# tky823/ssspy

Hardware: AMD Instinct MI355X
Metric: GaussILRMA-IP1 update_once mixture-iterations/sec (F=1025,T=512,N=4,K=16) (higher is better)
Workload: dtype f64; 1 GPU; BASELINE configs[1] GaussILRMA-IP1/MM (N=M=4, F=1025, T=512, n_basis=16) x 128 independent mixtures per GPU (configs[4] shard), record_loss=False, update_once() = one fused C-ABI call; batch_per_gpu=128, global_batch=128, n_bins=1025, n_frames=512, n_basis=16, parallelism=mixtures sharded, no collective, input=nmf_mixture(seed=1000+b) per mixture b (SURVEY 8d)

## Files before the change

### include/ssspy_amd.h

```cpp
#ifndef SSSPY_AMD_H
#define SSSPY_AMD_H

#include <stddef.h>

#ifdef __cplusplus
extern "C" {
#endif

enum {
  SSSPY_OK = 0,
  SSSPY_ERR_BADARG = 1,
  SSSPY_ERR_HIP = 2,
  SSSPY_ERR_UNSUPPORTED = 3,
  SSSPY_ERR_INTERNAL = 4,
};

enum { SSSPY_FLOOR_NONE = 0, SSSPY_FLOOR_MAX = 1, SSSPY_FLOOR_ADD = 2 };

enum {
  SSSPY_WEIGHT_UNIT = 0,
  SSSPY_WEIGHT_FRAME = 1,
  SSSPY_WEIGHT_BIN_FRAME = 2,
};

// ... 185 lines not shown
int ssspy_ilrma_deferred_logdet_slots(int B, int N, int F, int T, int K, double domain,
                                      int source_model);
int ssspy_ilrma_ip1_update_loss_slots(const void *X, const void *C, void *W, double *basis,
                                      double *activation, void *U, int B, int N, int F, int T,
                                      int K, double domain, int source_model, double model_param,
                                      int normalize, int floor_kind, double floor_eps,
                                      void *workspace, size_t workspace_bytes, int *info,
                                      double *slots, long long slot_stride, double *logdet,
                                      void *stream);
size_t ssspy_fold_scalar_slots_workspace_bytes(long long total, int nslots);
int ssspy_fold_scalar_slots(const double *slots, long long total, int nslots, double *out,
                            void *workspace, size_t workspace_bytes, void *stream);

enum {
  SSSPY_ROUTE_LATENCY = 0,
  SSSPY_ROUTE_THROUGHPUT = 1,
  SSSPY_ROUTE_GROUPED = 2,
  SSSPY_ROUTE_GENERIC = 3,
  SSSPY_ROUTE_WIDE_BASIS = 4,
  SSSPY_ROUTE_RUNTIME_N = 5,
};
int ssspy_ilrma_route(int B, int N, int F, int T, int K, double domain, int source_model,
                      int *act_chunks, int *basis_plan);

int ssspy_ipa_sweep(void *Vc, void *G, int B, int F, int N, int normalization, int max_iter,
                    int floor_kind, double floor_eps, int *info, void *newton_ws,
                    int *not_converged, void *stream);
size_t ssspy_ipa_sweep_newton_words(int B, int N);
int ssspy_debug_barrier_timeouts(void);

int ssspy_ilrma_partition_expand(const double *basis, const double *activation,
                                 const double *latent, double *Teff, double *Vrep, int B, int N,
                                 int F, int T, int K, void *stream);

enum { SSSPY_PARTITION_LATENT = 1, SSSPY_PARTITION_BASIS = 2, SSSPY_PARTITION_ACTIVATION = 4 };

int ssspy_ilrma_partition_update(const void *X, const void *W, double *basis, double *activation,
                                 double *latent, double *Teff, double *Vrep, int B, int N, int F,
                                 int T, int K, double domain, int source_model, double model_param,
                                 int steps, int floor_kind, double floor_eps, void *workspace,
                                 size_t workspace_bytes, void *stream);

int ssspy_ilrma_partition_normalize(void *W, const void *C, void *Y, double *basis, double *latent,
                                    int B, int N, int F, int T, int K, double domain,
                                    int floor_kind, double floor_eps, void *workspace,
                                    size_t workspace_bytes, void *stream);
// ... 585 lines not shown
```

### ssspy_amd/_lib.py

```python

import ctypes
import os

import numpy as np

_PKG = os.path.dirname(os.path.abspath(__file__))
LIB_PATH = os.environ.get("SSSPY_AMD_LIB") or os.path.join(_PKG, "lib", "libssspy_amd.so")

OK, ERR_BADARG, ERR_HIP, ERR_UNSUPPORTED, ERR_INTERNAL = 0, 1, 2, 3, 4
FLOOR_NONE, FLOOR_MAX, FLOOR_ADD = 0, 1, 2
WEIGHT_UNIT, WEIGHT_FRAME, WEIGHT_BIN_FRAME = 0, 1, 2
SOURCE_GAUSS, SOURCE_T, SOURCE_GGD = 0, 1, 2
PARTITION_LATENT, PARTITION_BASIS, PARTITION_ACTIVATION = 1, 2, 4
SOURCE_ME = 0x100
CONTRAST_LAPLACE, CONTRAST_GAUSS, CONTRAST_GAUSS_FIXED = 0, 1, 2
WHITEN, PCA_FIRST_COMPONENT_LAST, PCA_FIRST_COMPONENT_FIRST = 0, 1, 2
IPSDTA_QUAD, IPSDTA_BASIS, IPSDTA_ACT, IPSDTA_COV = range(4)
IPSDTA_MAX_SOURCES, IPSDTA_MAX_BLOCK, IPSDTA_MAX_BASIS = 8, 8, 32
(ROUTE_LATENCY, ROUTE_THROUGHPUT, ROUTE_GROUPED, ROUTE_GENERIC, ROUTE_WIDE_BASIS,
 ROUTE_RUNTIME_N) = range(6)
MNMF_ROUTE_TILED, MNMF_ROUTE_GENERIC, MNMF_ROUTE_RUNTIME = range(3)
MNMF_PLAN_FIELDS = ("fast", "ksmall", "basis_copy", "glds_cov", "glds_spatial", "kq", "handover",
                    "tail_full", "tail_tail", "tail_split", "tail_groups", "htail_full", "htail_tail",
                    "htail_split", "htail_groups", "act_chunks", "ip1_records", "spatial_fold_in_norm",
# ... 81 lines not shown
    "ssspy_ilrma_weighted_covariance": (_i, [_p, _p, _p, _p, _p, _i, _i, _i, _i, _i, _d, _i, _d, _i,
                                             _d, _p, _z, _p]),
    "ssspy_ilrma_normalize_filter": (_i, [_p, _p, _p, _i, _i, _i, _i, _d, _i, _d, _p, _z, _p]),
    "ssspy_ilrma_normalize_output": (_i, [_p, _p, _p, _i, _i, _i, _i, _i, _d, _i, _d, _p, _z, _p]),
    "ssspy_ilrma_normalize_output_tracked": (_i, [_p, _p, _p, _i, _i, _i, _i, _i, _d, _i, _d, _p, _z,
                                                  _p, _p]),
    "ssspy_ilrma_iss_weight": (_i, [_p, _p, _p, _p, _i, _i, _i, _i, _i, _d, _i, _d, _i, _d, _p]),
    "ssspy_ilrma_iss_weight_power": (_i, [_p, _p, _p, _p, _i, _i, _i, _i, _i, _d, _i, _d, _i, _d, _p]),
    "ssspy_ilrma_loss_workspace_bytes": (_z, [_i, _i, _i, _i, _i, _i]),
    "ssspy_ilrma_loss_data": (_i, [_p, _p, _p, _p, _p, _i, _i, _i, _i, _i, _d, _i, _d, _p, _z, _p]),
    "ssspy_ilrma_ip1_update": (_i, [_p, _p, _p, _p, _p, _p, _i, _i, _i, _i, _i, _d, _i, _d, _i, _i, _d,
                                    _p, _z, _p, _p]),
    "ssspy_ilrma_deferred_loss_supported": (_i, [_i, _i, _i, _i, _d, _i]),
    "ssspy_ilrma_ip1_update_deferred_loss": (_i, [_p, _p, _p, _p, _p, _p, _i, _i, _i, _i, _i, _d, _i,
                                                  _d, _i, _i, _d, _p, _z, _p, _p, _p, _p]),
    "ssspy_ilrma_deferred_loss_slots": (_i, [_i, _i, _i, _i, _i, _d, _i]),
    "ssspy_ilrma_deferred_logdet_slots": (_i, [_i, _i, _i, _i, _i, _d, _i]),
    "ssspy_ilrma_ip1_update_loss_slots": (_i, [_p, _p, _p, _p, _p, _p, _i, _i, _i, _i, _i, _d, _i,
                                               _d, _i, _i, _d, _p, _z, _p, _p, _q, _p, _p]),
    "ssspy_fold_scalar_slots_workspace_bytes": (_z, [_q, _i]),
    "ssspy_fold_scalar_slots": (_i, [_p, _q, _i, _p, _p, _z, _p]),
    "ssspy_ilrma_route": (_i, [_i, _i, _i, _i, _i, _d, _i, ctypes.POINTER(ctypes.c_int),
                                ctypes.POINTER(ctypes.c_int)]),
    "ssspy_ilrma_partition_expand": (_i, [_p, _p, _p, _p, _p, _i, _i, _i, _i, _i, _p]),
    "ssspy_ilrma_partition_update": (_i, [_p, _p, _p, _p, _p, _p, _p, _i, _i, _i, _i, _i, _d, _i, _d,
                                          _i, _i, _d, _p, _z, _p]),
    "ssspy_ilrma_partition_normalize": (_i, [_p, _p, _p, _p, _p, _i, _i, _i, _i, _i, _d, _i, _d, _p,
                                             _z, _p]),
    "ssspy_iva_frame_power_workspace_bytes": (_z, [_i, _i, _i, _i]),
    "ssspy_iva_frame_power": (_i, [_p, _p, _p, _i, _i, _i, _i, _p, _z, _p]),
    "ssspy_separate_frame_power": (_i, [_p, _p, _p, _p, _i, _i, _i, _i, _p, _z, _p]),
    "ssspy_iva_weight": (_i, [_p, _p, _p, _i, _i, _i, _i, _i, _i, _d, _p]),
    "ssspy_iva_loss_data": (_i, [_p, _p, _p, _i, _i, _i, _i, _i, _p]),
    "ssspy_overiva_frame_power_workspace_bytes": (_z, [_i, _i, _i, _i]),
    "ssspy_overiva_frame_power": (_i, [_p, _p, _q, _p, _p, _i, _i, _i, _i, _i, _p, _z, _p]),
    "ssspy_overiva_step_workspace_bytes": (_z, [_i, _i]),
    "ssspy_overiva_step": (_i, [_p, _p, _p, _i, _i, _i, _i, _i, _d, _p, _p, _p, _p, _z, _p]),
    "ssspy_iva_score_weight": (_i, [_p, _p, _p, _i, _i, _i, _i, _i, _i, _d, _p]),
    "ssspy_iva_grad_step_logdet_slots": (_i, [_i, _i, _i]),
    "ssspy_iva_grad_step": (_i, [_p, _p, _i, _i, _i, _i, _i, _i, _d, _p, _p, _q, _p]),
    "ssspy_fdica_weight": (_i, [_p, _p, _i, _i, _i, _i, _i, _i, _d, _p, _q, _p]),
    "ssspy_fdica_route": (_i, [_i, _i, _i, _i, _i]),
    "ssspy_fdica_steps": (_i, [_p, _p, _i, _i, _i, _i, _i, _i, _d, _i, _d, _i, _p, _p, _q, _p, _p]),
    "ssspy_wpe_route": (_i, [_i, _i, _i, _i, _i, ctypes.POINTER(ctypes.c_int)]),
    "ssspy_wpe_steps": (_i, [_p, _p, _p, _i, _i, _i, _i, _i, _i, _i, _d, _i, _p, _q, _p, _i, _p]),
    "ssspy_wpe_step": (_i, [_p, _p, _p, _i, _i, _i, _i, _i, _i, _i, _d, _p, _p, _p, _p, _p, _i, _p]),
# ... 182 lines not shown
```

### ssspy_amd/_ops.py

```python

from . import _device as dv
from . import _lib, _routes
from ._device import ptr


def _L():
    return _lib.load()


import os as _os

_CANARY_DOUBLES = 4096 if _os.environ.get("SSSPY_AMD_WS_CANARY") else 0
_CANARY_VALUE = -7.25e300
_canaries = []


def _workspace(nbytes, dev):
    n = (int(nbytes) + 7) // 8
    buf = dv.empty((n + _CANARY_DOUBLES,), dv.f64, dev)
    if not _CANARY_DOUBLES:
        return buf, int(nbytes)
    import weakref

    buf[n:].fill_(_CANARY_VALUE)
# ... 499 lines not shown
        ptr(X), ptr(C), ptr(W), ptr(basis), ptr(activation), ptr(U), B, N, F, T, K, domain, model[0],
        model[1], int(bool(normalize)), flooring[0], flooring[1], ptr(ws), ws_bytes, ptr(info),
        ptr(slots), int(slot_stride), ptr(logdet), _st()), "ilrma_ip1_update_loss_slots")


def fold_scalar_slots(slots, total, nslots, out):
    ws, ws_bytes = _scratch(_L().ssspy_fold_scalar_slots_workspace_bytes(int(total), int(nslots)),
                            slots.device)
    _lib.check(_L().ssspy_fold_scalar_slots(ptr(slots), int(total), int(nslots), ptr(out), ptr(ws),
                                            ws_bytes, _st()), "fold_scalar_slots")
    return out


def ilrma_route(B, N, F, T, K, domain, model=GAUSS):
    import ctypes

    chunks = ctypes.c_int(0)
    plan = (ctypes.c_int * 3)()
    route = int(_L().ssspy_ilrma_route(B, N, F, T, K, float(domain), model[0], ctypes.byref(chunks),
                                       plan))
    if route < 0:
        raise ValueError("ilrma_route: bad shape")
    return route, int(chunks.value), tuple(plan)


def ilrma_partition_expand(basis, activation, latent, Teff, Vrep):
    B, N, F, K = Teff.shape
    T = Vrep.shape[-1]
    _lib.check(
        _L().ssspy_ilrma_partition_expand(ptr(basis), ptr(activation), ptr(latent), ptr(Teff),
                                          ptr(Vrep), B, N, F, T, K, _st()),
        "ilrma_partition_expand",
    )


def ilrma_partition_update(X, W, basis, activation, latent, Teff, Vrep, domain, steps, flooring, ws,
                           ws_bytes, model=GAUSS):
    B, N, F, T = X.shape
    K = basis.shape[-1]
    _lib.check(
        _L().ssspy_ilrma_partition_update(ptr(X), ptr(W), ptr(basis), ptr(activation), ptr(latent),
                                          ptr(Teff), ptr(Vrep), B, N, F, T, K, domain, model[0],
                                          model[1], steps, flooring[0], flooring[1], ptr(ws),
                                          ws_bytes, _st()),
        "ilrma_partition_update",
    )
# ... 1328 lines not shown
```

### ssspy_amd/csrc/ilrma_api.hip

```cpp
#include "ilrma_plan.hpp"

namespace ssspy {

static inline int check_model(int source_model, double param, double domain = 2.0) {
  const int model = source_model & 0xff;
  const bool me = (source_model & SSSPY_SOURCE_ME) != 0;
  if ((source_model & ~(0xff | SSSPY_SOURCE_ME)) != 0)
    return fail(SSSPY_ERR_BADARG, "bad source model flags");
  if (me && (domain != 2.0 || model == SSSPY_SOURCE_GGD))
    return fail(SSSPY_ERR_BADARG, "ME source updates need domain == 2 and a Gauss or t model");
  if (model == SSSPY_SOURCE_GAUSS) return SSSPY_OK;
  if (model == SSSPY_SOURCE_T && param > 0.0) return SSSPY_OK;
  if (model == SSSPY_SOURCE_GGD && param > 0.0 && param < 2.0) return SSSPY_OK;
  return fail(SSSPY_ERR_BADARG, "bad source model / model_param (t: dof > 0, GGD: 0 < beta < 2)");
}

int ip1_with_power(void *W, const void *U, const void *C, double *qbuf, int B, int F, int N,
                   int floor_kind, double floor_eps, int *info, hipStream_t st);
int separate_power(const void *X, const void *W, double *P, int B, int N, int F, int T,
                   hipStream_t st);
int row_power(const void *W, const void *C, double *qbuf, int B, int F, int N, hipStream_t st);
int wb_update_basis(const double *a, const double *b, double *basis, const double *activation,
                    double *nd, int BN, int F, int T, int K, const IlrmaDims &d, hipStream_t st);
int wb_update_activation(const double *a, const double *b, const double *basis, double *activation,
// ... 772 lines not shown
    int split = 0, rbins = 0;
    auto cov = [&]() -> int {
      ILRMA_FAST_DISPATCH(N, ilrma_fast_wcov, X, W, basis, activation, U, B, F, T, K, ws + w.upart,
                          p.fm_id, p.fm_param, floor_kind, floor_eps, st, &split, &rbins);
    };
    rc = cov();
    if (rc) return rc;
    auto ip1 = [&]() -> int {
      if (loss_data && loss_stride > 0) {
        ILRMA_FAST_DISPATCH(N, ilrma_small_ip1_logdet,
                            split ? (const void *)(ws + w.upart) : (const void *)U, split, rbins, 0ll,
                            normalize ? C : nullptr, W, B, F, floor_kind, floor_eps, qbuf, info,
                            logdet, loss_stride, st);
      }
      ILRMA_FAST_DISPATCH(N, ilrma_small_ip1, split ? (const void *)(ws + w.upart) : (const void *)U,
                          split, rbins, 0ll, normalize ? C : nullptr, W, B, F, floor_kind, floor_eps,
                          qbuf, info, st);
    };
    rc = ip1();
    if (rc || !normalize) return rc;
    ILRMA_FAST_DISPATCH(N, ilrma_small_norm, W, basis, qbuf, B, F, K, domain, floor_kind, floor_eps,
                        st);
  }
  rc = wcov_into(p, w, d, X, W, basis, activation, U, ws, p.power_once ? Xs : nullptr, p.power_once,
                 st);
  if (rc) return rc;
  rc = ip1_with_power(W, U, normalize ? C : nullptr, normalize ? qbuf : nullptr, B, F, N,
                      floor_kind, floor_eps, info, st);
  if (rc || !normalize) return rc;
  return launch_norm_scale(W, basis, qbuf, B, N, F, K, domain, floor_kind, floor_eps, st);
}

int ssspy_ilrma_ip1_update(const void *X, const void *C, void *W, double *basis, double *activation,
                           void *U, int B, int N, int F, int T, int K, double domain,
                           int source_model, double model_param, int normalize, int floor_kind,
                           double floor_eps, void *workspace, size_t workspace_bytes, int *info,
                           void *stream) {
  return ip1_update_impl(X, C, W, basis, activation, U, B, N, F, T, K, domain, source_model,
                         model_param, normalize, floor_kind, floor_eps, workspace, workspace_bytes,
                         info, nullptr, nullptr, stream);
}

int ssspy_ilrma_deferred_loss_supported(int N, int F, int T, int K, double domain,
                                        int source_model) {
  return make_ilrma_plan(1, N, F, T, K, domain, source_model).loss_byproduct;
}
// ... 27 lines not shown
                                      void *workspace, size_t workspace_bytes, int *info,
                                      double *slots, long long slot_stride, double *logdet,
                                      void *stream) {
  SSSPY_REQUIRE(slots && logdet && slot_stride >= B && slot_stride < (1ll << 31),
                "ilrma_ip1_update_loss_slots: bad argument");
  return ip1_update_impl(X, C, W, basis, activation, U, B, N, F, T, K, domain, source_model,
                         model_param, normalize, floor_kind, floor_eps, workspace, workspace_bytes,
                         info, slots, logdet, stream, slot_stride);
}

int ssspy_ilrma_route(int B, int N, int F, int T, int K, double domain, int source_model,
                      int *chunks_out, int *basis_plan) {
  if (B <= 0 || N < 2 || N > SSSPY_RT_MAX_SOURCES || F <= 0 || T <= 0 || K < 1 ||
      K > SSSPY_MAX_BASIS || !(domain > 0.0 && domain <= 2.0))
    return -1;
  const IlrmaPlan p = make_ilrma_plan(B, N, F, T, K, domain, source_model);
  if (chunks_out) *chunks_out = p.act_chunks;
  if (basis_plan) {
    basis_plan[0] = p.basis_tail.full;
    basis_plan[1] = p.basis_tail.tail;
    basis_plan[2] = p.basis_tail.split;
  }
  return p.summary;
}

size_t ssspy_fold_scalar_slots_workspace_bytes(long long total, int nslots) {
  if (total <= 0 || nslots <= 0) return 0;
  return align256(fold_scratch_bytes(total, nslots)) + 256;
}

int ssspy_fold_scalar_slots(const double *slots, long long total, int nslots, double *out,
                            void *workspace, size_t workspace_bytes, void *stream) {
  SSSPY_REQUIRE(slots && out && total > 0 && nslots > 0, "fold_scalar_slots: bad argument");
  SSSPY_REQUIRE(workspace && workspace_bytes >= ssspy_fold_scalar_slots_workspace_bytes(total, nslots),
                "fold_scalar_slots: workspace too small");
  return launch_fold_slabs(slots, workspace, out, total, nslots, as_stream(stream), 0);
}

int ssspy_ilrma_partition_expand(const double *basis, const double *activation,
                                 const double *latent, double *Teff, double *Vrep, int B, int N,
                                 int F, int T, int K, void *stream) {
  SSSPY_REQUIRE(basis && activation && latent && Teff && Vrep && B > 0 && N >= 1 && F > 0 &&
                    T > 0 && K >= 1,
                "partition_expand: bad argument");
  const long long per = (long long)K * (F > T ? F : T);
  hipLaunchKernelGGL(k_partition_expand, dim3((unsigned)((per + 255) / 256), N, B), dim3(256), 0,
// ... 106 lines not shown
```

### ssspy_amd/csrc/ilrma_fast.hip

```cpp
#include <cstdlib>

#include "common.hpp"
#include "cov_core.hpp"
#include "fast_model.hpp"
#include "fast_tiles.hpp"
#include "tail_plan.hpp"

#ifndef SSSPY_N
#error "compile with -DSSSPY_N=<n_sources>"
#endif
#if SSSPY_N > 4
#error "fast path is built for n_sources <= 4"
#endif

#define SSSPY_CAT_(a, b) a##b
#define SSSPY_CAT(a, b) SSSPY_CAT_(a, b)
#define LAUNCHER(name) SSSPY_CAT(SSSPY_CAT(name, _n), SSSPY_N)

namespace ssspy {
namespace SSSPY_CAT(ilrma_fast_n, SSSPY_N) {

constexpr int N = SSSPY_N;
using fast::rcp_nr;
using fast::FastModel;
using fast::FM_GAUSS;
using fast::FM_GAUSS1;
using fast::FM_GAUSSP;
using fast::FM_GGD;
// ... 431 lines not shown
}

template <int G>
__device__ __forceinline__ void wc_half_tile(double (&acc)[4][WC_HALF], const c128 *patch,
                                             const double *shared, int lane, int c, int q) {
#pragma unroll
  for (int r = 0; r < 4; ++r) {
    c128 x[4];
#pragma unroll
    for (int m = 0; m < 4; ++m) x[m] = patch[(m * 16 + c) * 17 + q + 4 * r];
    double phi[4];
#pragma unroll
    for (int n = 0; n < 4; ++n)
      phi[n] = shared[(n * 4 + r) * 64 + lane];
    double v[WC_HALF];
    wc_half_terms<G>(x, v);
#pragma unroll
    for (int n = 0; n < 4; ++n)
#pragma unroll
      for (int e = 0; e < WC_HALF; ++e) acc[n][e] = fma(phi[n], v[e], acc[n][e]);
  }
}

template <int G>
__device__ __forceinline__ void wc_half_store(const double (&acc)[4][WC_HALF], c128 *dst,
                                              double scale) {
  constexpr int PA[2][4][2] = {{{0, 1}, {2, 3}, {0, 0}, {0, 0}}, {{0, 2}, {0, 3}, {1, 2}, {1, 3}}};
  constexpr int NPAIR = G == 0 ? 2 : 4, P0 = G == 0 ? 4 : 0;
#pragma unroll
  for (int n = 0; n < 4; ++n) {
    c128 *d = dst + n * 16;
    if constexpr (G == 0) {
#pragma unroll
      for (int a = 0; a < 4; ++a) d[a * 4 + a] = cmake(acc[n][a] * scale, 0.0);
    }
#pragma unroll
    for (int p = 0; p < NPAIR; ++p) {
      const int a = PA[G][p][0], bb = PA[G][p][1];
      const double zx = acc[n][P0 + 2 * p], zy = acc[n][P0 + 2 * p + 1];
      d[a * 4 + bb] = cmake(zx * scale, zy * scale);
      d[bb * 4 + a] = cmake(zx * scale, -zy * scale);
    }
  }
}

template <int MODEL, int KS, bool FULL = false>
__global__ __launch_bounds__(256, KS >= 16 ? 1 : 2) void k_wcov_fast(const c128 *__restrict__ X,
                                                      const c128 *__restrict__ W,
                                                      const double *__restrict__ basis,
                                                      const double *__restrict__ act,
                                                      c128 *__restrict__ U, int F, int T, int K,
                                                      TailPlan plan, c128 *__restrict__ upart,
                                                      FastModel fm) {
  constexpr int SG = WC_SG;
  constexpr int WSTRIDE = N * N + 1;
  __shared__ __attribute__((aligned(16))) c128 xpatch[4][XPATCH];
  constexpr bool NEEDS_Y = MODEL == FM_T || MODEL == FM_GGD;
  __shared__ __attribute__((aligned(16))) c128 wlc[NEEDS_Y ? 4 * 16 * WSTRIDE : 1];
  constexpr bool SPLIT = WC_SHARE && !NEEDS_Y && MODEL != FM_GAUSSP && KS == 4;
  __shared__ __attribute__((aligned(16))) double phis[SPLIT ? WC_WB * N * 4 * 64 : 1];
  const int lane = threadIdx.x & 63, wave = threadIdx.x >> 6;
  const int c = lane & 15, q = lane >> 4;
  const BlockWork work = block_work(plan);
  const int b = work.b, nchunks = work.nchunks;
  const int g = wave % WC_NG, wb = wave / WC_NG;
  const int s0 = g * SG;
  const int i0 = (work.group * WC_WB + wb) * 16;
  const int bin = min(i0 + c, F - 1);
  const fast::XSrc<N> xsrc = fast::make_xsrc<N>(X + (long long)b * N * F * T, F, T);
  c128 *xshare = &xpatch[0][0] + wb * (N * 16 * 17);
  const double *act_b = act + (long long)b * N * K * T;
  const int ntiles = (T + 15) >> 4;
  const int tpc = (ntiles + nchunks - 1) / nchunks;
  const int jt_begin = work.chunk * tpc, jt_end = min(ntiles, jt_begin + tpc);
  if (wave_idle(i0, F)) {
    if (NEEDS_Y) __syncthreads();
    if constexpr (WC_SHARE) {
      for (int jt = jt_begin; jt < jt_end; ++jt) {
        __syncthreads();
        __syncthreads();
      }
    }
    return;
  }
  double tb[SG][KS];
#pragma unroll
  for (int s = 0; s < SG; ++s)
#pragma unroll
    for (int ks = 0; ks < KS; ++ks) {
      const int kk = 4 * ks + q, n = min(s0 + s, N - 1);
      tb[s][ks] = (FULL || kk < K) ? basis[(((long long)b * N + n) * F + bin) * K + kk] : 0.0;
    }
  c128 *wmine = wlc + (NEEDS_Y ? (wave * 16 + c) * WSTRIDE : 0);
  if (NEEDS_Y) {
    for (int e = lane; e < 16 * N * N; e += 64) {
      const int bl = e / (N * N), rem = e % (N * N);
      wlc[(wave * 16 + bl) * WSTRIDE + rem] = W[((long long)b * F + min(i0 + bl, F - 1)) * (N * N) + rem];
    }
  }
  CovAcc<N, SPLIT ? 1 : SG> acc;
  double hacc[SPLIT ? 4 : 1][WC_HALF];
  if constexpr (SPLIT) {
#pragma unroll
    for (int n = 0; n < 4; ++n)
#pragma unroll
// ... 92 lines not shown
    }
  }
  const double scale = 1.0 / (double)T;
  const int ob = i0 + c;
  auto out_bin = [&]() -> c128 * {
    return nchunks == 1 ? U + ((long long)b * F + ob) * (long long)(N * N * N)
                        : upart + (((long long)work.tail_idx * nchunks + work.chunk) * WC_BINS +
                                   (ob - work.group * WC_BINS)) * (long long)(N * N * N);
  };
  if constexpr (SPLIT) {
#pragma unroll
    for (int n = 0; n < 4; ++n)
#pragma unroll
      for (int e = 0; e < WC_HALF; ++e) {
        double v = hacc[n][e];
        v += __shfl_xor(v, 16, 64);
        v += __shfl_xor(v, 32, 64);
        hacc[n][e] = v;
      }
    if (ob < F && q == 0) {
      c128 *dst = out_bin();
      if (gu == 0) wc_half_store<0>(hacc, dst, scale);
      else wc_half_store<1>(hacc, dst, scale);
    }
    return;
  }
  acc.fold_q();
  if (ob < F) {
    c128 *dst = out_bin();
#pragma unroll
    for (int s = 0; s < SG; ++s) {
      const int n = s0 + s;
      if (n < N) {
        int e = 0;
#pragma unroll
        for (int a = 0; a < N; ++a) {
          const bool mine = (a & 3) == q;
          if (mine) dst[(n * N + a) * N + a] = cmake(acc.diag[s][a] * scale, 0.0);
#pragma unroll
          for (int bb = a + 1; bb < N; ++bb) {
            const c128 z = acc.off[s][e];
            if (mine) {
              dst[(n * N + a) * N + bb] = cmake(z.x * scale, z.y * scale);
              dst[(n * N + bb) * N + a] = cmake(z.x * scale, -z.y * scale);
            }
            ++e;
// ... 62 lines not shown
  if (ob < F) {
    c128 *dst = U + ((long long)b * F + ob) * (long long)(N * N * N);
#pragma unroll
    for (int s = 0; s < SG; ++s) {
      const int n = s0 + s;
      if (n < N) {
        int e = 0;
#pragma unroll
        for (int a = 0; a < N; ++a) {
          const bool mine = (a & 3) == q;
          if (mine) dst[(n * N + a) * N + a] = cmake(acc.diag[s][a] * scale, 0.0);
#pragma unroll
          for (int bb = a + 1; bb < N; ++bb) {
            const c128 z = acc.off[s][e];
            if (mine) {
              dst[(n * N + a) * N + bb] = cmake(z.x * scale, z.y * scale);
              dst[(n * N + bb) * N + a] = cmake(z.x * scale, -z.y * scale);
            }
            ++e;
          }
        }
      }
    }
  }
}

__global__ __launch_bounds__(256) void k_wcov_fold(c128 *__restrict__ U,
                                                   const c128 *__restrict__ upart, int F,
                                                   TailPlan plan) {
  constexpr int PER = WC_BINS * N * N * N;
  const int tail_idx = blockIdx.y;
  const int item = plan.full + tail_idx;
  const int b = item / plan.groups, group = item - b * plan.groups;
  const int e = blockIdx.x * blockDim.x + threadIdx.x;
  const int lb = e / (N * N * N);
  if (e >= PER || group * WC_BINS + lb >= F) return;
  const c128 s2 = ordered_sum(upart + (long long)tail_idx * plan.split * PER + e, (long long)PER,
                              plan.split);
  U[((long long)b * F + group * WC_BINS) * (long long)(N * N * N) + e] = s2;
}

template <int KS>
struct TStage {
  double t[(N * 16 * 4 * KS + 255) / 256];
  c128 w;
};
// ... 393 lines not shown
  const int nslots = plan.groups * (plan.split > 1 ? plan.split : 1) * 4;
  int rc = scalar_slots_begin(loss_ws, B, nslots, st);
  if (rc) return rc;
  double *slots = (double *)loss_ws;
  SSSPY_FAST_LAUNCH2(k_loss_fast, W != nullptr, (const c128 *)X, (const c128 *)W,
                     basis, act, slots, F, T, K, plan, fm, B);
  rc = check_launch("k_loss_fast");
  return rc ? rc : scalar_slots_fold(loss_ws, B, nslots, out, 0, st);
}

int LAUNCHER(ilrma_fast_wcov)(const void *X, const void *W, const double *basis, const double *act,
                              void *U, int B, int F, int T, int K, void *upart, int fmodel,
                              double mparam, int floor_kind, double floor_eps, hipStream_t st,
                              int *split_out = nullptr, int *rbins_out = nullptr) {
  if (split_out) *split_out = 0;
  if (rbins_out) *rbins_out = WC_BINS;
  const TailPlan plan =
      make_tail_plan(B, (F + WC_BINS - 1) / WC_BINS, (T + 15) / 16, K > 32 ? 256 : SLOTS,
                     K > 32 ? 256 : 1024);
  const FastModel fm = make_fast_model(fmodel, mparam, 0, floor_kind, floor_eps);
  dim3 grid(plan.full + plan.tail * plan.split), block(256);
#define SSSPY_WCOV_LAUNCH_F(M, KS_, FULL_)                                                        \
  hipLaunchKernelGGL((k_wcov_fast<M, KS_, FULL_>), grid, block, 0, st, (const c128 *)X,            \
                     (const c128 *)W, basis, act, (c128 *)U, F, T, K, plan, (c128 *)upart, fm)
#define SSSPY_WCOV_LAUNCH(M, KS_) SSSPY_WCOV_LAUNCH_F(M, KS_, false)
#define SSSPY_WCOV_LAUNCH_M(KS_)                       \
  switch (fmodel) {                                    \
    case FM_T: SSSPY_WCOV_LAUNCH(FM_T, KS_); break;    \
    case FM_GGD: SSSPY_WCOV_LAUNCH(FM_GGD, KS_); break; \
    case FM_GAUSS1: SSSPY_WCOV_LAUNCH(FM_GAUSS1, KS_); break; \
    case FM_GAUSSP: SSSPY_WCOV_LAUNCH(FM_GAUSSP, KS_); break; \
    default: SSSPY_WCOV_LAUNCH(FM_GAUSS, KS_); break;  \
  }
  if (K > 32) {
    SSSPY_WCOV_LAUNCH_M(16)
  } else if (K > 16) {
    SSSPY_WCOV_LAUNCH_M(8)
  } else if (full_tiles(K, T) && fmodel == FM_GAUSS) {
    SSSPY_WCOV_LAUNCH_F(FM_GAUSS, 4, true);
  } else {
    SSSPY_WCOV_LAUNCH_M(4)
  }
#undef SSSPY_WCOV_LAUNCH_M
#undef SSSPY_WCOV_LAUNCH
#undef SSSPY_WCOV_LAUNCH_F
  int rc = check_launch("k_wcov_fast");
  if (rc || plan.tail == 0) return rc;
  if (split_out && plan.full == 0) {
    *split_out = plan.split;
    return rc;
  }
  hipLaunchKernelGGL(k_wcov_fold, dim3((WC_BINS * N * N * N + 255) / 256, plan.tail), block, 0, st,
                     (c128 *)U, (const c128 *)upart, F, plan);
  return check_launch("k_wcov_fold");
}

int LAUNCHER(ilrma_fast_wcov_frame)(const void *X, const double *weight, void *U, int B, int F,
                                    int T, hipStream_t st) {
  static const bool disabled = std::getenv("SSSPY_AMD_NO_FAST") != nullptr;
  const int groups = (F + WC_BINS - 1) / WC_BINS;
  const long long items = (long long)B * groups;
  if (disabled || items < SLOTS || (long long)F * T * 16 >= (1ll << 32)) return -1;
  hipLaunchKernelGGL(k_wcov_frame_fast, dim3((unsigned)items), dim3(256), 0, st, (const c128 *)X,
                     weight, (c128 *)U, F, T, groups);
  return check_launch("k_wcov_frame_fast");
}

#endif

#undef SSSPY_FAST_LAUNCH2
#undef SSSPY_FAST_LAUNCH_M

}
```

### ssspy_amd/csrc/ilrma_plan.hpp

```cpp
#pragma once

#include <cstdlib>

#include "common.hpp"
#include "ilrma_params.hpp"
#include "tail_plan.hpp"
#include "wide_n.hpp"

namespace ssspy {

#define DECL_N(n)                                                                               \
  int ilrma_basis_n##n(const void *, const void *, const double *, double *, const double *,   \
                       IlrmaDims, hipStream_t);                                                \
  int ilrma_activation_n##n(const void *, const void *, const double *, const double *, double *, \
                            int, IlrmaDims, hipStream_t);                                      \
  int ilrma_wcov_n##n(const void *, const void *, const double *, const double *, void *,       \
                      IlrmaDims, hipStream_t);                                                 \
  size_t ilrma_loss_ws_bytes_n##n(int, int);                                                   \
  int ilrma_loss_n##n(const void *, const void *, const double *, const double *, double *,     \
                      void *, IlrmaDims, hipStream_t);
DECL_N(2) DECL_N(3) DECL_N(4) DECL_N(5) DECL_N(6) DECL_N(7) DECL_N(8)
#undef DECL_N

#define DECL_FAST(n)                                                                           \
  int ilrma_fast_basis_n##n(const void *, const void *, const double *, double *, const double *, \
                            int, int, int, int, int, double, double *, int, double, int,        \
                            double *, void *, int, hipStream_t, long long);                     \
  int ilrma_fast_basis_loss_slots_n##n(int, int, int);                                          \
  size_t ilrma_fast_loss_ws_bytes_n##n(int, int);                                               \
  int ilrma_fast_activation_n##n(const void *, const void *, const double *, double *,         \
                                 double *, int, int, int, int, int, int, double, int,           \
                                 hipStream_t, int *, int, int, double);                         \
  int ilrma_fast_wcov_n##n(const void *, const void *, const double *, const double *, void *, \
                           int, int, int, int, void *, int, double, int, double, hipStream_t,  \
                           int *, int *);                                                      \
  int ilrma_fast_loss_n##n(const void *, const void *, const double *, const double *, double *, \
                           void *, int, int, int, int, int, double, hipStream_t);
DECL_FAST(2) DECL_FAST(3) DECL_FAST(4)
#undef DECL_FAST

#define DECL_SMALL(n)                                                                           \
  size_t ilrma_small_scratch_n##n(int, int, int, int);                                            \
  int ilrma_small_activation_n##n(const void *, const void *, const double *, double *, int, int, \
                                  int, int, int, double, double *, int, double, int,              \
                                  hipStream_t);                                                   \
  int ilrma_small_ip1_n##n(const void *, int, int, long long, const void *, void *, int, int, int, \
                           double, double *, int *, hipStream_t);                                 \
  int ilrma_small_ip1_logdet_n##n(const void *, int, int, long long, const void *, void *, int,   \
                                  int, int, double, double *, int *, double *, long long,         \
                                  hipStream_t);                                                   \
  int ilrma_small_norm_n##n(void *, double *, const double *, int, int, int, double, int, double, \
                            hipStream_t);
DECL_SMALL(2) DECL_SMALL(3) DECL_SMALL(4)
#undef DECL_SMALL

bool wide_weighted_cov_ok(int N, int S, int F, int T, int kind);
int wide_weighted_cov(const void *A, const double *weight, int kind, void *U, int B, int N, int S,
                      int F, int T, hipStream_t st);
size_t wb_loss_ws_bytes(int B, int N, int F, int T);

#define ILRMA_FAST_DISPATCH(N_, fn, ...)             \
  switch (N_) {                                      \
    case 2: return fn##_n2(__VA_ARGS__);             \
    case 3: return fn##_n3(__VA_ARGS__);             \
    default: return fn##_n4(__VA_ARGS__);            \
  }
#define ILRMA_DISPATCH_OR(N_, otherwise, fn, ...)                                    \
  switch (N_) {                                                                      \
    case 2: return fn##_n2(__VA_ARGS__);                                             \
    case 3: return fn##_n3(__VA_ARGS__);                                             \
    case 4: return fn##_n4(__VA_ARGS__);                                             \
    case 5: return fn##_n5(__VA_ARGS__);                                             \
    case 6: return fn##_n6(__VA_ARGS__);                                             \
    case 7: return fn##_n7(__VA_ARGS__);                                             \
    case 8: return fn##_n8(__VA_ARGS__);                                             \
    default: return otherwise;                                                       \
  }
#define ILRMA_DISPATCH(N_, fn, ...)                                                               \
  ILRMA_DISPATCH_OR(N_, fail(SSSPY_ERR_UNSUPPORTED, "ILRMA: n_sources must be in [2, 8]"), fn, \
                    __VA_ARGS__)

static inline bool tuned_sources(int N) { return N >= 2 && N <= 4; }
// ... 92 lines not shown
enum class CovRoute { RuntimeN, WideBasis, MatrixCore, Tuned, Generic };

struct IlrmaPlan {
  int N, K;
  int fm_id, me;
  double fm_param;
  bool gauss;
  NmfRoute nmf;
  SourceRun runs[3];
  int nruns;
  int act_chunks;
  bool act_latency;
  bool act_in_place;
  bool basis_out_of_place;
  TailPlan basis_tail;
  LossRoute loss;
  bool loss_byproduct;
  int loss_slots, logdet_slots;
  bool runtime_n;
  bool cov_matrix_core;
  bool cov_tuned;
  bool power_once;
  bool ip1_latency;
  bool weights_buf;
  bool dense_buf;
  int summary;
};

static inline IlrmaPlan make_ilrma_plan(int B, int N, int F, int T, int K, double domain,
                                        int source_model, double model_param = 0.0) {
  IlrmaPlan p;
  p.N = N;
  p.K = K;
  p.fm_id = fast_model_id(domain, source_model);
  p.fm_param = p.fm_id == 4 ? domain : model_param;
  p.me = (source_model & SSSPY_SOURCE_ME) ? 1 : 0;
  p.gauss = (source_model & 0xff) == SSSPY_SOURCE_GAUSS;
  const bool fast = fast_path(N, F, T, K, domain, source_model);
  const bool small = small_path(B, N, F, T, K, domain, source_model);
  const bool wide = wide_basis_shape(N, K);
  p.nruns = source_runs(B, N, F, T, K, domain, source_model, p.runs);
  p.nmf = p.nruns               ? NmfRoute::Grouped
          : (fast && K <= 32)   ? NmfRoute::Tuned
          : wide                ? NmfRoute::WideBasis
                                : NmfRoute::Generic;
  const bool tuned = p.nmf == NmfRoute::Tuned;
  p.act_chunks = act_chunks(B, N, F, T, K);
  p.act_latency = small;
#ifdef SSSPY_NO_ACT_INPLACE
  p.act_in_place = false;
#else
  p.act_in_place = tuned && p.act_chunks == 1 && K <= 16;
#endif
  p.basis_out_of_place = K > 16;
  p.basis_tail = tuned ? ilrma_basis_plan(B, F, T, K) : TailPlan{0, 0, 1, 0};
  p.runtime_n = rt_sources_ok(N);
  p.loss = (fast && K <= 16)           ? LossRoute::Tuned
           : (K > 16 || p.runtime_n)   ? LossRoute::WideBasis
                                       : LossRoute::Generic;
  p.loss_byproduct = p.loss == LossRoute::Tuned && p.fm_id != 1;
  p.loss_slots = p.loss_byproduct ? tuned_basis_loss_slots(B, N, F, T) : 0;
  p.logdet_slots = p.loss_byproduct ? (small ? (F + 15) / 16 : 1) : 0;
  p.cov_matrix_core = N > 4 && wide_weighted_cov_ok(N, N, F, T, SSSPY_WEIGHT_BIN_FRAME);
  p.cov_tuned = fast;
  p.power_once = p.nmf == NmfRoute::Grouped || p.nmf == NmfRoute::WideBasis;
  p.ip1_latency = small;
  p.weights_buf = N > 4 || wide;
  p.dense_buf = wide;
  p.summary = p.runtime_n                      ? SSSPY_ROUTE_RUNTIME_N
              : p.nmf == NmfRoute::Grouped     ? SSSPY_ROUTE_GROUPED
              : small                          ? SSSPY_ROUTE_LATENCY
              : p.nmf == NmfRoute::WideBasis   ? SSSPY_ROUTE_WIDE_BASIS
              : tuned                          ? SSSPY_ROUTE_THROUGHPUT
                                               : SSSPY_ROUTE_GENERIC;
  return p;
}

static inline CovRoute cov_route(const IlrmaPlan &p, bool ysep, bool filter) {
  const bool weights_ok = p.gauss || ysep || !filter;
  if (p.runtime_n) return CovRoute::RuntimeN;
  if (p.K > 32 && weights_ok) return CovRoute::WideBasis;
  if (p.cov_matrix_core && weights_ok) return CovRoute::MatrixCore;
  if (p.cov_tuned && (p.gauss || filter)) return CovRoute::Tuned;
  return CovRoute::Generic;
}

static inline IlrmaPlan shape_plan(int B, int N, int F, int T, int K) {
  return make_ilrma_plan(B, N, F, T, K, 2.0, SSSPY_SOURCE_GAUSS);
}
// ... 56 lines not shown
```

Measured before the change: 42390 iterations/s.

## Fuse the IP1 demixing update into the weighted covariance kernel epilogue

For the tuned Gauss N=4 route, the weighted covariance kernel now stages each bin's U matrices in shared memory and runs the IP1 row solve in place, writing W and the normalisation powers directly. Bins handled by split tail tiles are finished by a separate small kernel after the fold. This removes the round trip of U through global memory and the separate IP1 launch. In exchange it adds extra barriers and shared-memory reuse inside the covariance kernel, plus a new per-row pivoting solver built from lane shuffles.

```diff
diff --git a/include/ssspy_amd.h b/include/ssspy_amd.h
--- a/include/ssspy_amd.h
+++ b/include/ssspy_amd.h
@@ -231,6 +231,8 @@
 };
 int ssspy_ilrma_route(int B, int N, int F, int T, int K, double domain, int source_model,
                       int *act_chunks, int *basis_plan);
+int ssspy_ilrma_ip1_route(int B, int N, int F, int T, int K, double domain, int source_model,
+                          int *cov_plan);
 
 int ssspy_ipa_sweep(void *Vc, void *G, int B, int F, int N, int normalization, int max_iter,
                     int floor_kind, double floor_eps, int *info, void *newton_ws,
diff --git a/ssspy_amd/_lib.py b/ssspy_amd/_lib.py
--- a/ssspy_amd/_lib.py
+++ b/ssspy_amd/_lib.py
@@ -127,6 +127,7 @@
     "ssspy_fold_scalar_slots": (_i, [_p, _q, _i, _p, _p, _z, _p]),
     "ssspy_ilrma_route": (_i, [_i, _i, _i, _i, _i, _d, _i, ctypes.POINTER(ctypes.c_int),
                                 ctypes.POINTER(ctypes.c_int)]),
+    "ssspy_ilrma_ip1_route": (_i, [_i, _i, _i, _i, _i, _d, _i, ctypes.POINTER(ctypes.c_int)]),
     "ssspy_ilrma_partition_expand": (_i, [_p, _p, _p, _p, _p, _i, _i, _i, _i, _i, _p]),
     "ssspy_ilrma_partition_update": (_i, [_p, _p, _p, _p, _p, _p, _p, _i, _i, _i, _i, _i, _d, _i, _d,
                                           _i, _i, _d, _p, _z, _p]),
diff --git a/ssspy_amd/_ops.py b/ssspy_amd/_ops.py
--- a/ssspy_amd/_ops.py
+++ b/ssspy_amd/_ops.py
@@ -545,6 +545,16 @@
     if route < 0:
         raise ValueError("ilrma_route: bad shape")
     return route, int(chunks.value), tuple(plan)
+
+
+def ilrma_ip1_route(B, N, F, T, K, domain, model=GAUSS):
+    import ctypes
+
+    plan = (ctypes.c_int * 3)()
+    epi = int(_L().ssspy_ilrma_ip1_route(B, N, F, T, K, float(domain), model[0], plan))
+    if epi < 0:
+        raise ValueError("ilrma_ip1_route: bad shape")
+    return bool(epi), tuple(plan)
 
 
 def ilrma_partition_expand(basis, activation, latent, Teff, Vrep):
diff --git a/ssspy_amd/csrc/ilrma_api.hip b/ssspy_amd/csrc/ilrma_api.hip
--- a/ssspy_amd/csrc/ilrma_api.hip
+++ b/ssspy_amd/csrc/ilrma_api.hip
@@ -818,6 +818,12 @@
     ILRMA_FAST_DISPATCH(N, ilrma_small_norm, W, basis, qbuf, B, F, K, domain, floor_kind, floor_eps,
                         st);
   }
+  if (p.cov_ip1_epilogue) {
+    rc = ilrma_fast_wcov_ip1_n4(X, W, normalize ? C : nullptr, basis, activation, U, B, F, T, K,
+                                ws + w.upart, p.fm_id, floor_kind, floor_eps, qbuf, info, st);
+    if (rc || !normalize) return rc;
+    return launch_norm_scale(W, basis, qbuf, B, N, F, K, domain, floor_kind, floor_eps, st);
+  }
   rc = wcov_into(p, w, d, X, W, basis, activation, U, ws, p.power_once ? Xs : nullptr, p.power_once,
                  st);
   if (rc) return rc;
@@ -891,6 +897,18 @@
     basis_plan[2] = p.basis_tail.split;
   }
   return p.summary;
+}
+
+int ssspy_ilrma_ip1_route(int B, int N, int F, int T, int K, double domain, int source_model,
+                          int *cov_plan) {
+  if (ssspy_ilrma_route(B, N, F, T, K, domain, source_model, nullptr, nullptr) < 0) return -1;
+  const IlrmaPlan p = make_ilrma_plan(B, N, F, T, K, domain, source_model);
+  if (cov_plan) {
+    cov_plan[0] = p.cov_tail.full;
+    cov_plan[1] = p.cov_tail.tail;
+    cov_plan[2] = p.cov_tail.split;
+  }
+  return p.cov_ip1_epilogue ? 1 : 0;
 }
 
 size_t ssspy_fold_scalar_slots_workspace_bytes(long long total, int nslots) {
diff --git a/ssspy_amd/csrc/ilrma_fast.hip b/ssspy_amd/csrc/ilrma_fast.hip
--- a/ssspy_amd/csrc/ilrma_fast.hip
+++ b/ssspy_amd/csrc/ilrma_fast.hip
@@ -4,6 +4,7 @@
 #include "cov_core.hpp"
 #include "fast_model.hpp"
 #include "fast_tiles.hpp"
+#include "ip1_rows_exact.hpp"
 #include "tail_plan.hpp"
 
 #ifndef SSSPY_N
@@ -481,14 +482,14 @@
   }
 }
 
-template <int G>
+template <int G, int NS = 16>
 __device__ __forceinline__ void wc_half_store(const double (&acc)[4][WC_HALF], c128 *dst,
                                               double scale) {
   constexpr int PA[2][4][2] = {{{0, 1}, {2, 3}, {0, 0}, {0, 0}}, {{0, 2}, {0, 3}, {1, 2}, {1, 3}}};
   constexpr int NPAIR = G == 0 ? 2 : 4, P0 = G == 0 ? 4 : 0;
 #pragma unroll
   for (int n = 0; n < 4; ++n) {
-    c128 *d = dst + n * 16;
+    c128 *d = dst + n * NS;
     if constexpr (G == 0) {
 #pragma unroll
       for (int a = 0; a < 4; ++a) d[a * 4 + a] = cmake(acc[n][a] * scale, 0.0);
@@ -503,20 +504,32 @@
   }
 }
 
-template <int MODEL, int KS, bool FULL = false>
+struct Ip1Epi {
+  c128 *W;
+  const c128 *C;
+  double *qbuf;
+  int *info;
+  int floor_kind;
+  double eps;
+};
+constexpr int EPI_NS = N * N + 1;
+
+template <int MODEL, int KS, bool FULL = false, bool EPI = false>
 __global__ __launch_bounds__(256, KS >= 16 ? 1 : 2) void k_wcov_fast(const c128 *__restrict__ X,
                                                       const c128 *__restrict__ W,
                                                       const double *__restrict__ basis,
                                                       const double *__restrict__ act,
                                                       c128 *__restrict__ U, int F, int T, int K,
                                                       TailPlan plan, c128 *__restrict__ upart,
-                                                      FastModel fm) {
+                                                      FastModel fm, Ip1Epi epi) {
   constexpr int SG = WC_SG;
   constexpr int WSTRIDE = N * N + 1;
   __shared__ __attribute__((aligned(16))) c128 xpatch[4][XPATCH];
   constexpr bool NEEDS_Y = MODEL == FM_T || MODEL == FM_GGD;
   __shared__ __attribute__((aligned(16))) c128 wlc[NEEDS_Y ? 4 * 16 * WSTRIDE : 1];
   constexpr bool SPLIT = WC_SHARE && !NEEDS_Y && MODEL != FM_GAUSSP && KS == 4;
+  static_assert(!EPI || (SPLIT && N == 4), "the IP1 epilogue rides on the component-split form");
+  static_assert(!EPI || WC_BINS * N * EPI_NS <= 4 * XPATCH, "the U stage fits the x patches");
   __shared__ __attribute__((aligned(16))) double phis[SPLIT ? WC_WB * N * 4 * 64 : 1];
   const int lane = threadIdx.x & 63, wave = threadIdx.x >> 6;
   const int c = lane & 15, q = lane >> 4;
@@ -540,6 +553,12 @@
         __syncthreads();
       }
     }
+    if constexpr (EPI) {
+      if (nchunks == 1) {
+        __syncthreads();
+        __syncthreads();
+      }
+    }
     return;
   }
   double tb[SG][KS];
@@ -678,6 +697,34 @@
       c128 *dst = out_bin();
       if (gu == 0) wc_half_store<0>(hacc, dst, scale);
       else wc_half_store<1>(hacc, dst, scale);
+    }
+    if constexpr (EPI) {
+      if (nchunks != 1) return;
+      c128 *ustage = &xpatch[0][0];
+      __syncthreads();
+      if (ob < F && q == 0) {
+        c128 *dst = ustage + (wb * 16 + c) * (N * EPI_NS);
+        if (gu == 0) wc_half_store<0, EPI_NS>(hacc, dst, scale);
+        else wc_half_store<1, EPI_NS>(hacc, dst, scale);
+      }
+      __syncthreads();
+      if (threadIdx.x >= 4 * WC_BINS) return;
+      const int bl = threadIdx.x >> 2, r = threadIdx.x & 3;
+      const int ebin = work.group * WC_BINS + bl;
+      const bool live = ebin < F;
+      const int bs = live ? bl : 0;
+      const long long gb = (long long)b * F + work.group * WC_BINS + bs;
+      c128 Wr[N];
+#pragma unroll
+      for (int cc = 0; cc < N; ++cc) Wr[cc] = epi.W[gb * (N * N) + r * N + cc];
+      const bool ok = ip1_rows_exact<N>(Wr, ustage + bs * (N * EPI_NS), EPI_NS, r, epi.floor_kind,
+                                        epi.eps);
+      if (live) {
+#pragma unroll
+        for (int cc = 0; cc < N; ++cc) epi.W[gb * (N * N) + r * N + cc] = Wr[cc];
+        if (!ok && epi.info && r == 0) atomicAdd(epi.info, 1);
+        if (epi.C && epi.qbuf) epi.qbuf[gb * N + r] = row_power_exact<N>(Wr, epi.C + gb * (N * N));
+      }
     }
     return;
   }
@@ -786,6 +833,26 @@
         }
       }
     }
+  }
+}
+
+__global__ __launch_bounds__(256) void k_ip1_tail(Ip1Epi epi, const c128 *__restrict__ U,
+                                                  long long bin0, long long nbins) {
+  const long long idx = bin0 + (((long long)blockIdx.x * 256 + threadIdx.x) >> 2);
+  const int r = threadIdx.x & 3;
+  const bool live = idx < nbins;
+  const long long gb = live ? idx : nbins - 1;
+  const bool row = r < N;
+  const int rr = row ? r : N - 1;
+  c128 Wr[N];
+#pragma unroll
+  for (int c = 0; c < N; ++c) Wr[c] = epi.W[gb * (N * N) + rr * N + c];
+  const bool ok = ip1_rows_exact<N>(Wr, U + gb * (N * N * N), N * N, r, epi.floor_kind, epi.eps);
+  if (live && row) {
+#pragma unroll
+    for (int c = 0; c < N; ++c) epi.W[gb * (N * N) + r * N + c] = Wr[c];
+    if (!ok && epi.info && r == 0) atomicAdd(epi.info, 1);
+    if (epi.C && epi.qbuf) epi.qbuf[gb * N + r] = row_power_exact<N>(Wr, epi.C + gb * (N * N));
   }
 }
 
@@ -1225,7 +1292,8 @@
   dim3 grid(plan.full + plan.tail * plan.split), block(256);
 #define SSSPY_WCOV_LAUNCH_F(M, KS_, FULL_)                                                        \
   hipLaunchKernelGGL((k_wcov_fast<M, KS_, FULL_>), grid, block, 0, st, (const c128 *)X,            \
-                     (const c128 *)W, basis, act, (c128 *)U, F, T, K, plan, (c128 *)upart, fm)
+                     (const c128 *)W, basis, act, (c128 *)U, F, T, K, plan, (c128 *)upart, fm,      \
+                     Ip1Epi{})
 #define SSSPY_WCOV_LAUNCH(M, KS_) SSSPY_WCOV_LAUNCH_F(M, KS_, false)
 #define SSSPY_WCOV_LAUNCH_M(KS_)                       \
   switch (fmodel) {                                    \
@@ -1256,6 +1324,60 @@
   hipLaunchKernelGGL(k_wcov_fold, dim3((WC_BINS * N * N * N + 255) / 256, plan.tail), block, 0, st,
                      (c128 *)U, (const c128 *)upart, F, plan);
   return check_launch("k_wcov_fold");
+}
+
+int LAUNCHER(ilrma_fast_wcov_ip1)(const void *X, void *W, const void *C, const double *basis,
+                                  const double *act, void *U, int B, int F, int T, int K,
+                                  void *upart, int fmodel, int floor_kind, double floor_eps,
+                                  double *qbuf, int *info, hipStream_t st) {
+#if SSSPY_N == 4
+  const TailPlan plan = make_tail_plan(B, (F + WC_BINS - 1) / WC_BINS, (T + 15) / 16, SLOTS, 1024);
+  if (fmodel != FM_GAUSS || K > 16 || plan.full == 0)
+    return fail(SSSPY_ERR_UNSUPPORTED, "ilrma_fast_wcov_ip1: shape outside the epilogue's route");
+  const FastModel fm = make_fast_model(fmodel, 0.0, 0, floor_kind, floor_eps);
+  const Ip1Epi epi{(c128 *)W, (const c128 *)C, C ? qbuf : nullptr, info, floor_kind, floor_eps};
+  dim3 grid(plan.full + plan.tail * plan.split), block(256);
+#ifdef SSSPY_IP1_ROWS_ONLY
+  if (full_tiles(K, T)) {
+    hipLaunchKernelGGL((k_wcov_fast<FM_GAUSS, 4, true, false>), grid, block, 0, st, (const c128 *)X,
+                       (const c128 *)W, basis, act, (c128 *)U, F, T, K, plan, (c128 *)upart, fm, epi);
+  } else {
+    hipLaunchKernelGGL((k_wcov_fast<FM_GAUSS, 4, false, false>), grid, block, 0, st, (const c128 *)X,
+                       (const c128 *)W, basis, act, (c128 *)U, F, T, K, plan, (c128 *)upart, fm, epi);
+  }
+  if (int rc0 = check_launch("k_wcov_fast")) return rc0;
+  if (plan.tail > 0)
+    hipLaunchKernelGGL(k_wcov_fold, dim3((WC_BINS * N * N * N + 255) / 256, plan.tail), block, 0, st,
+                       (c128 *)U, (const c128 *)upart, F, plan);
+  {
+    const long long nb = (long long)B * F;
+    hipLaunchKernelGGL(k_ip1_tail, dim3((unsigned)((nb * 4 + 255) / 256)), block, 0, st, epi,
+                       (const c128 *)U, 0ll, nb);
+    return check_launch("k_ip1_tail");
+  }
+#endif
+  if (full_tiles(K, T)) {
+    hipLaunchKernelGGL((k_wcov_fast<FM_GAUSS, 4, true, true>), grid, block, 0, st, (const c128 *)X,
+                       (const c128 *)W, basis, act, (c128 *)U, F, T, K, plan, (c128 *)upart, fm, epi);
+  } else {
+    hipLaunchKernelGGL((k_wcov_fast<FM_GAUSS, 4, false, true>), grid, block, 0, st, (const c128 *)X,
+                       (const c128 *)W, basis, act, (c128 *)U, F, T, K, plan, (c128 *)upart, fm, epi);
+  }
+  int rc = check_launch("k_wcov_fast");
+  if (rc || plan.tail == 0) return rc;
+  hipLaunchKernelGGL(k_wcov_fold, dim3((WC_BINS * N * N * N + 255) / 256, plan.tail), block, 0, st,
+                     (c128 *)U, (const c128 *)upart, F, plan);
+  rc = check_launch("k_wcov_fold");
+  if (rc) return rc;
+  const long long nbins = (long long)B * F;
+  const long long bin0 = (long long)(plan.full / plan.groups) * F +
+                         (long long)(plan.full % plan.groups) * WC_BINS;
+  hipLaunchKernelGGL(k_ip1_tail, dim3((unsigned)(((nbins - bin0) * 4 + 255) / 256)), block, 0, st, epi,
+                     (const c128 *)U, bin0, nbins);
+  return check_launch("k_ip1_tail");
+#else
+  return fail(SSSPY_ERR_UNSUPPORTED, "ilrma_fast_wcov_ip1: built for 4 sources");
+#endif
 }
 
 int LAUNCHER(ilrma_fast_wcov_frame)(const void *X, const double *weight, void *U, int B, int F,
diff --git a/ssspy_amd/csrc/ilrma_plan.hpp b/ssspy_amd/csrc/ilrma_plan.hpp
--- a/ssspy_amd/csrc/ilrma_plan.hpp
+++ b/ssspy_amd/csrc/ilrma_plan.hpp
@@ -35,7 +35,10 @@
                            int, int, int, int, void *, int, double, int, double, hipStream_t,  \
                            int *, int *);                                                      \
   int ilrma_fast_loss_n##n(const void *, const void *, const double *, const double *, double *, \
-                           void *, int, int, int, int, int, double, hipStream_t);
+                           void *, int, int, int, int, int, double, hipStream_t);                \
+  int ilrma_fast_wcov_ip1_n##n(const void *, void *, const void *, const double *, const double *, \
+                               void *, int, int, int, int, void *, int, int, double, double *,    \
+                               int *, hipStream_t);
 DECL_FAST(2) DECL_FAST(3) DECL_FAST(4)
 #undef DECL_FAST
 
@@ -58,6 +61,7 @@
 int wide_weighted_cov(const void *A, const double *weight, int kind, void *U, int B, int N, int S,
                       int F, int T, hipStream_t st);
 size_t wb_loss_ws_bytes(int B, int N, int F, int T);
+bool ip1_small_shape(int B, int F, int N);
 
 #define ILRMA_FAST_DISPATCH(N_, fn, ...)             \
   switch (N_) {                                      \
@@ -196,6 +200,8 @@
   bool cov_tuned;
   bool power_once;
   bool ip1_latency;
+  bool cov_ip1_epilogue;
+  TailPlan cov_tail;
   bool weights_buf;
   bool dense_buf;
   int summary;
@@ -239,6 +245,15 @@
   p.cov_tuned = fast;
   p.power_once = p.nmf == NmfRoute::Grouped || p.nmf == NmfRoute::WideBasis;
   p.ip1_latency = small;
+  p.cov_tail = (tuned && N == 4 && K <= 32)
+                   ? make_tail_plan(B, (F + 31) / 32, (T + 15) / 16, SLOTS, 1024)
+                   : TailPlan{0, 0, 1, 0};
+#ifdef SSSPY_NO_IP1_EPILOGUE
+  p.cov_ip1_epilogue = false;
+#else
+  p.cov_ip1_epilogue = tuned && N == 4 && K <= 16 && p.fm_id == 0 && !small &&
+                       !ip1_small_shape(B, F, N) && p.cov_tail.full > 0;
+#endif
   p.weights_buf = N > 4 || wide;
   p.dense_buf = wide;
   p.summary = p.runtime_n                      ? SSSPY_ROUTE_RUNTIME_N
diff --git a/ssspy_amd/csrc/ip1_rows_exact.hpp b/ssspy_amd/csrc/ip1_rows_exact.hpp
--- /dev/null
+++ b/ssspy_amd/csrc/ip1_rows_exact.hpp
@@ -0,0 +1,134 @@
+#pragma once
+
+#include "common.hpp"
+
+namespace ssspy {
+namespace ip1_exact {
+
+enum { F_RE = 1, F_IM = 2, X_RE = 4, X_IM = 8, Q_U = 16, Q_C = 32 };
+
+template <bool SECOND>
+__device__ __forceinline__ double mul_re(c128 a, c128 b) {
+  return SECOND ? fma(a.x, b.x, -(a.y * b.y)) : fma(-a.y, b.y, a.x * b.x);
+}
+template <bool SECOND>
+__device__ __forceinline__ double mul_im(c128 a, c128 b) {
+  return SECOND ? fma(a.x, b.y, a.y * b.x) : fma(a.y, b.x, a.x * b.y);
+}
+template <bool SECOND>
+__device__ __forceinline__ double herm_term(c128 w, c128 t) {
+  return SECOND ? fma(w.x, t.x, w.y * t.y) : fma(w.y, t.y, w.x * t.x);
+}
+
+}
+
+#ifndef SSSPY_IP1_EXACT_FORMS
+#define SSSPY_IP1_EXACT_FORMS (ip1_exact::F_RE | ip1_exact::X_RE | ip1_exact::Q_U | ip1_exact::Q_C)
+#endif
+
+template <int N, int FORMS = SSSPY_IP1_EXACT_FORMS>
+__device__ __forceinline__ bool ip1_rows_exact(c128 (&Wr)[N], const c128 *Ub, int ustride, int r,
+                                               int floor_kind, double eps) {
+  using namespace ip1_exact;
+  constexpr int G = 4;
+  static_assert(N <= G, "one lane per row");
+  const bool row = r < N;
+  const int rr = row ? r : N - 1;
+  bool ok = true;
+#pragma unroll 1
+  for (int n = 0; n < N; ++n) {
+    const c128 *Un = Ub + n * ustride;
+    c128 a[N];
+#pragma unroll
+    for (int c = 0; c < N; ++c) a[c] = cmake(0.0, 0.0);
+#pragma unroll
+    for (int m = 0; m < N; ++m)
+#pragma unroll
+      for (int c = 0; c < N; ++c) cfma(a[c], Wr[m], Un[m * N + c]);
+    c128 rhs = cmake(r == n ? 1.0 : 0.0, 0.0);
+    int own[N];
+#pragma unroll
+    for (int p = 0; p < N; ++p) own[p] = p;
+    int order = row ? -1 : N;
+    c128 pinv[N];
+#pragma unroll
+    for (int k = 0; k < N; ++k) {
+      const double mag = cabs1(a[k]);
+      double v[N];
+#pragma unroll
+      for (int p = k; p < N; ++p) v[p] = __shfl(mag, own[p], G);
+#pragma unroll
+      for (int p = k + 1; p < N; ++p) {
+        const bool sw = v[p] > v[k];
+        const double vk = v[k], vp = v[p];
+        const int ok_ = own[k], op = own[p];
+        v[k] = sw ? vp : vk;
+        v[p] = sw ? vk : vp;
+        own[k] = sw ? op : ok_;
+        own[p] = sw ? ok_ : op;
+      }
+      const int pl = own[k];
+      if (r == pl) order = k;
+      c128 prow[N];
+#pragma unroll
+      for (int c = k; c < N; ++c) prow[c] = cmake(__shfl(a[c].x, pl, G), __shfl(a[c].y, pl, G));
+      const c128 prhs = cmake(__shfl(rhs.x, pl, G), __shfl(rhs.y, pl, G));
+      const c128 piv = prow[k];
+      ok = ok && (piv.x != 0.0 || piv.y != 0.0);
+      pinv[k] = crecip(piv);
+      if (order < 0) {
+        const c128 f = cmake(mul_re<(FORMS & F_RE) != 0>(a[k], pinv[k]),
+                             mul_im<(FORMS & F_IM) != 0>(a[k], pinv[k]));
+#pragma unroll
+        for (int c = k + 1; c < N; ++c) cfms(a[c], f, prow[c]);
+        cfms(rhs, f, prhs);
+      }
+    }
+    c128 w[N];
+#pragma unroll
+    for (int k = N - 1; k >= 0; --k) {
+      c128 acc = rhs;
+#pragma unroll
+      for (int j = k + 1; j < N; ++j) cfms(acc, a[j], w[j]);
+      const c128 mine = cmake(mul_re<(FORMS & X_RE) != 0>(acc, pinv[k]),
+                              mul_im<(FORMS & X_IM) != 0>(acc, pinv[k]));
+      w[k] = cmake(__shfl(mine.x, own[k], G), __shfl(mine.y, own[k], G));
+    }
+    c128 t = cmake(0.0, 0.0);
+#pragma unroll
+    for (int b2 = 0; b2 < N; ++b2) cfma(t, Un[rr * N + b2], w[b2]);
+    double term = 0.0;
+#pragma unroll
+    for (int c = 0; c < N; ++c)
+      if (c == rr) term = herm_term<(FORMS & Q_U) != 0>(w[c], t);
+    double qf = 0.0;
+#pragma unroll
+    for (int c = 0; c < N; ++c) qf += __shfl(term, c, G);
+    qf = qf < 0.0 ? 0.0 : qf;
+    const double d = apply_floor(sqrt(qf), floor_kind, eps);
+    if (r == n) {
+#pragma unroll
+      for (int c = 0; c < N; ++c) Wr[c] = cmake(w[c].x / d, -w[c].y / d);
+    }
+  }
+  return ok;
+}
+
+template <int N, int FORMS = SSSPY_IP1_EXACT_FORMS>
+__device__ __forceinline__ double row_power_exact(const c128 (&Wr)[N], const c128 *Cm) {
+  using namespace ip1_exact;
+  c128 v[N];
+#pragma unroll
+  for (int m = 0; m < N; ++m) v[m] = cconj(Wr[m]);
+  double q = 0.0;
+#pragma unroll
+  for (int a2 = 0; a2 < N; ++a2) {
+    c128 t = cmake(0.0, 0.0);
+#pragma unroll
+    for (int b2 = 0; b2 < N; ++b2) cfma(t, Cm[a2 * N + b2], v[b2]);
+    q += herm_term<(FORMS & Q_C) != 0>(v[a2], t);
+  }
+  return q;
+}
+
+}
```

Result: slower. 41910 iterations/s (-1.1%).
